# preiter93/ndrustfft

Hardware: AMD Instinct MI355X
Metric: GFFT-points/s, batched 1-D C2C FFT f64 along the contiguous axis (+ achieved HBM GB/s vs roofline) (higher is better)
Workload: dtype f64

## Files before the change

### include/ndfft_mi355x.h

```cpp
#ifndef NDFFT_MI355X_H
#define NDFFT_MI355X_H

#include <stddef.h>
#include <stdint.h>

#ifdef __cplusplus
extern "C" {
#endif

#define NDFFT_ABI_VERSION 1
#define NDFFT_ABI_MINOR 6

typedef enum {
    NDFFT_OK = 0,
    NDFFT_ERR_INVALID_ARG = 1,
    NDFFT_ERR_SIZE_MISMATCH = 2,
    NDFFT_ERR_SHAPE_MISMATCH = 3,
    NDFFT_ERR_AXIS = 4,
    NDFFT_ERR_UNSUPPORTED = 5,
    NDFFT_ERR_HIP = 6,
    NDFFT_ERR_NO_DEVICE = 7,
    NDFFT_ERR_ALLOC = 8
} ndfft_status;

typedef enum { NDFFT_F32 = 0, NDFFT_F64 = 1 } ndfft_dtype;

typedef enum {
    NDFFT_KIND_C2C = 0,
    NDFFT_KIND_R2C = 1,
    NDFFT_KIND_DCT = 2
} ndfft_kind;

typedef enum {
    NDFFT_OP_C2C_FWD = 0,
    NDFFT_OP_C2C_INV = 1,
    NDFFT_OP_R2C = 2,
    NDFFT_OP_C2R = 3,
    NDFFT_OP_DCT1 = 4,
    NDFFT_OP_DCT2 = 5,
    NDFFT_OP_DCT3 = 6,
    NDFFT_OP_DCT4 = 7
} ndfft_op;

typedef enum { NDFFT_NORM_NONE = 0, NDFFT_NORM_DEFAULT = 1, NDFFT_NORM_SCALE = 2 } ndfft_norm;
// ... 70 lines not shown
```

### include/ndfft_mi355x_ext.h

```cpp
#ifndef NDFFT_MI355X_EXT_H
#define NDFFT_MI355X_EXT_H

#include "ndfft_mi355x.h"

#ifdef __cplusplus
extern "C" {
#endif

int ndfft_exec_weighted_device(const ndfft_plan *plan, int op, const void *d_in, void *d_out, int ndim,
                               const int64_t *shape_in, const int64_t *stride_in,
                               const int64_t *shape_out, const int64_t *stride_out,
                               int axis, const void *d_weights, size_t n_weights, void *stream);

#define NDFFT_FILTER_NO_FUSE 1
int ndfft_exec_filter_device(const ndfft_plan *plan, const void *d_in, void *d_out, int ndim,
                             const int64_t *shape, const int64_t *stride_in, const int64_t *stride_out, int axis,
                             const void *d_weights, size_t n_weights, int norm, double scale, int flags, void *stream);

int ndfft_exec_dct_filter_device(const ndfft_plan *plan, const void *d_in, void *d_out, int ndim,
                                 const int64_t *shape, const int64_t *stride_in, const int64_t *stride_out, int axis,
                                 const void *d_weights, size_t n_weights, int norm, double scale, int flags, void *stream);

#ifdef __cplusplus
}
#endif
#endif
```

### ndrustfft_amd/_lib.py

```python
import ctypes
import os

_HERE = os.path.dirname(os.path.abspath(__file__))
LIB_PATH = os.environ.get("NDFFT_MI355X_LIB") or os.path.join(_HERE, "csrc", "libndfft_mi355x.so")

OK, ERR_INVALID_ARG, ERR_SIZE_MISMATCH, ERR_SHAPE_MISMATCH, ERR_AXIS, ERR_UNSUPPORTED, ERR_HIP, ERR_NO_DEVICE, ERR_ALLOC = range(9)
F32, F64 = 0, 1
KIND_C2C, KIND_R2C, KIND_DCT = 0, 1, 2
OP_C2C_FWD, OP_C2C_INV, OP_R2C, OP_C2R, OP_DCT1, OP_DCT2, OP_DCT3, OP_DCT4 = range(8)
NORM_NONE, NORM_DEFAULT, NORM_SCALE = 0, 1, 2
INPUT_AUTO, INPUT_CACHED, INPUT_COLD = 0, 1, 2

SYMBOLS = [
    "ndfft_abi_version", "ndfft_abi_minor", "ndfft_last_error", "ndfft_device_count", "ndfft_set_device",
    "ndfft_plan_create", "ndfft_plan_retain", "ndfft_plan_destroy", "ndfft_plan_n", "ndfft_plan_kind",
    "ndfft_plan_dtype", "ndfft_plan_lane_len_in", "ndfft_plan_lane_len_out",
    "ndfft_exec", "ndfft_exec_device", "ndfft_exec_sharded", "ndfft_exec_sharded_device", "ndfft_last_path", "ndfft_explain_plan",
    "ndfft_dev_alloc", "ndfft_dev_free", "ndfft_dev_upload", "ndfft_dev_download", "ndfft_dev_sync",
    "ndfft_release_workspace", "ndfft_host_alloc", "ndfft_host_free", "ndfft_set_input_hint", "ndfft_host_forget", "ndfft_host_reg_cache", "ndfft_last_input_policy",
    "ndfft_documented_switches", "ndfft_reload_switches", "ndfft_jit_prebuild",
]
EXT_SYMBOLS = ["ndfft_exec_weighted_device"]
FILTER_SYMBOLS = ["ndfft_exec_filter_device"]
FILTER_NO_FUSE = 1
DCT_FILTER_SYMBOLS = ["ndfft_exec_dct_filter_device"]


_loaded = []


class NdfftError(RuntimeError):
    def __init__(self, status, msg):
        super().__init__(msg)
        self.status = status


class Panic(NdfftError):
    """A condition on which the reference panics (size / axis / Zip mismatch); message text matches."""


class Library:
    def __init__(self, path=LIB_PATH):
        if not os.path.exists(path):
            raise ImportError(
                f"{path} not found: build it with `make -C ndrustfft_amd/csrc` (or __graft_entry__.build()). "
                "ndrustfft_amd has no CPU fallback.")
        self.path = path
        L = self.c = ctypes.CDLL(path)
        _loaded.append(self)
        vp, i32, sz, i64p, dbl = ctypes.c_void_p, ctypes.c_int, ctypes.c_size_t, ctypes.c_void_p, ctypes.c_double
        L.ndfft_abi_version.restype = i32
        L.ndfft_abi_minor.restype = i32
        L.ndfft_last_error.restype = ctypes.c_char_p
        L.ndfft_last_path.restype = ctypes.c_char_p
        L.ndfft_explain_plan.argtypes = [ctypes.c_int, ctypes.c_int, ctypes.c_size_t, ctypes.c_char_p, ctypes.c_size_t]
        L.ndfft_explain_plan.restype = ctypes.c_int
        L.ndfft_device_count.restype = i32
        L.ndfft_set_device.argtypes = [i32]
# ... 16 lines not shown
        L.ndfft_dev_upload.argtypes = [vp, vp, sz]
        L.ndfft_dev_download.argtypes = [vp, vp, sz]
        L.ndfft_dev_sync.argtypes = [vp]
        L.ndfft_release_workspace.argtypes = []; L.ndfft_release_workspace.restype = ctypes.c_int
        L.ndfft_host_alloc.argtypes = [ctypes.POINTER(vp), ctypes.c_size_t]; L.ndfft_host_alloc.restype = ctypes.c_int
        L.ndfft_host_free.argtypes = [vp]; L.ndfft_host_free.restype = ctypes.c_int
        L.ndfft_set_input_hint.argtypes = [i32]; L.ndfft_set_input_hint.restype = i32
        L.ndfft_host_forget.argtypes = [vp]; L.ndfft_host_forget.restype = i32
        L.ndfft_host_reg_cache.argtypes = [sz]; L.ndfft_host_reg_cache.restype = i32
        L.ndfft_last_input_policy.argtypes = []; L.ndfft_last_input_policy.restype = i32
        L.ndfft_documented_switches.argtypes = [ctypes.c_char_p, sz]; L.ndfft_documented_switches.restype = i32
        L.ndfft_reload_switches.argtypes = []; L.ndfft_reload_switches.restype = i32
        ip = ctypes.POINTER(ctypes.c_int)
        try:
            L.ndfft_jit_prebuild.argtypes = [ctypes.c_char_p, ctypes.c_char_p, i32, i32, ip, ip, ip]; L.ndfft_jit_prebuild.restype = i32
        except AttributeError:
            if not os.environ.get("NDFFT_MI355X_LIB"):
                raise
        try:
            L.ndfft_exec_weighted_device.argtypes = [vp, i32, vp, vp, i32, i64p, i64p, i64p, i64p, i32, vp, sz, vp]; L.ndfft_exec_weighted_device.restype = i32
        except AttributeError:
            if not os.environ.get("NDFFT_MI355X_LIB"):
                raise
        try:
            L.ndfft_exec_filter_device.argtypes = [vp, vp, vp, i32, i64p, i64p, i64p, i32, vp, sz, i32, dbl, i32, vp]; L.ndfft_exec_filter_device.restype = i32
        except AttributeError:
            if not os.environ.get("NDFFT_MI355X_LIB"):
                raise
        try:
            L.ndfft_exec_dct_filter_device.argtypes = [vp, vp, vp, i32, i64p, i64p, i64p, i32, vp, sz, i32, dbl, i32, vp]; L.ndfft_exec_dct_filter_device.restype = i32
        except AttributeError:
            if not os.environ.get("NDFFT_MI355X_LIB"):
                raise

    def check(self, status):
        if status == OK:
            return
        msg = self.c.ndfft_last_error().decode() or f"ndfft status {status}"
        if status in (ERR_SIZE_MISMATCH, ERR_SHAPE_MISMATCH, ERR_AXIS):
            raise Panic(status, msg)
        raise NdfftError(status, msg)

    def last_path(self):
        return self.c.ndfft_last_path().decode()

    def reload_switches(self):
        self.check(self.c.ndfft_reload_switches())

    def jit_prebuild(self, manifest, out_dir, first=0, stride=1):
        b, p, f = ctypes.c_int(0), ctypes.c_int(0), ctypes.c_int(0)
        self.check(self.c.ndfft_jit_prebuild(os.fsencode(manifest), os.fsencode(out_dir), first, stride, ctypes.byref(b), ctypes.byref(p), ctypes.byref(f)))
        return b.value, p.value, f.value

    def documented_switches(self):
        buf = ctypes.create_string_buffer(4096)
        self.c.ndfft_documented_switches(buf, len(buf))
        return buf.value.decode().split()

    def last_input_policy(self):
        return int(self.c.ndfft_last_input_policy())

    def explain_plan(self, kind, dtype, n):
        buf = ctypes.create_string_buffer(4096)
        need = self.c.ndfft_explain_plan(kind, dtype, n, buf, len(buf))
        if need < 0:
            raise NdfftError(-need, self.c.ndfft_last_error().decode())
        return buf.value.decode()


_default = None


def default():
    global _default
    if _default is None:
        _default = Library()
    return _default
```

### ndrustfft_amd/csrc/device_common.h

```cpp
#pragma once
#ifndef __HIPCC_RTC__
#include <hip/hip_runtime.h>
#include <stdint.h>
#else
typedef __hip_internal::int64_t int64_t;
typedef __hip_internal::int32_t int32_t;
typedef __hip_internal::uint32_t uint32_t;
typedef __hip_internal::uint64_t uint64_t;
#endif

namespace ndfft {

template <typename T> struct vec2;
typedef float ndfft_c32 __attribute__((ext_vector_type(2)));
template <> struct vec2<float> { using type = ndfft_c32; };
template <> struct vec2<double> { using type = double2; };
template <typename T> using cpx = typename vec2<T>::type;

template <typename T> __host__ __device__ inline cpx<T> mk(T a, T b) { cpx<T> r; r.x = a; r.y = b; return r; }
template <typename C> __host__ __device__ inline C cadd(C a, C b) { a.x += b.x; a.y += b.y; return a; }
template <typename C> __host__ __device__ inline C csub(C a, C b) { a.x -= b.x; a.y -= b.y; return a; }
template <typename C> __host__ __device__ inline C cmul(C a, C b) {
    C r; r.x = a.x * b.x - a.y * b.y; r.y = a.x * b.y + a.y * b.x; return r;
}
__host__ __device__ inline ndfft_c32 cadd(ndfft_c32 a, ndfft_c32 b) { return a + b; }
__host__ __device__ inline ndfft_c32 csub(ndfft_c32 a, ndfft_c32 b) { return a - b; }
__host__ __device__ inline ndfft_c32 cmul(ndfft_c32 a, ndfft_c32 b) { const ndfft_c32 bs = {-b.y, b.x}; return a.xx * b + a.yy * bs; }
template <typename C> __host__ __device__ inline C cconj(C a) { a.y = -a.y; return a; }
template <typename C> __host__ __device__ inline C cmul_mi(C a) { C r; r.x = a.y; r.y = -a.x; return r; }

enum GenOp : int {
    G_C2C_FWD = 0, G_C2C_INV,
    G_R2C_EVEN, G_R2C_ODD, G_C2R_EVEN, G_C2R_ODD,
    G_DCT1,
    G_DCT2_EVEN, G_DCT2_ODD, G_DCT3_EVEN, G_DCT3_ODD,
    G_DCT4_EVEN, G_DCT4_ODD
};

struct Pow2Args {
    const void *in; void *out;
    int64_t nlanes;
    int64_t pitch_in, pitch_out;
    int32_t inverse;
    double scale;
    const void *twp;
    const void *twlo = nullptr, *twhi = nullptr;
    int32_t logB = 0, f1 = 1;
    int32_t xcd_chunk = 0;
    int32_t stream_in = -1;
};

struct WaveArgs {
    const void *in; void *out;
    int64_t total;
    int32_t inverse;
    double scale;
    const void *tw;
    int32_t xcd_chunk;
};

struct TinyArgs {
    const void *in; void *out;
    int64_t nlanes;
    int64_t inner;
    int64_t outer_in, outer_out;
    int64_t lane_in, lane_out;
    int64_t elem_in, elem_out;
    int32_t inverse;
    double scale;
    const void *mat = nullptr;
};

struct RegRealArgs {
    TinyArgs t;
    const void *aux1, *aux2;
};

__device__ __forceinline__ unsigned xcd_block(unsigned b, unsigned nblk, int chunk) {
    if (chunk <= 0) return b;
    const unsigned grp = 8u * (unsigned)chunk;
    const unsigned g = b / grp;
    if ((g + 1) * grp > nblk) return b;
    const unsigned r = b - g * grp;
    return g * grp + (r & 7u) * (unsigned)chunk + (r >> 3);
}

}
```

### ndrustfft_amd/csrc/exec.hip

```cpp
#include <algorithm>
#include <atomic>
#include <mutex>
#include <cstdio>
#include <cstdlib>
#include <cstring>
#include <map>
#include <string>
#include <type_traits>

#include "exec_internal.h"
#include "pow2_real.h"
#include "../../include/ndfft_mi355x_ext.h"

namespace ndfft {

static int kind_of_op(int op) {
    if (op == NDFFT_OP_C2C_FWD || op == NDFFT_OP_C2C_INV) return NDFFT_KIND_C2C;
    if (op == NDFFT_OP_R2C || op == NDFFT_OP_C2R) return NDFFT_KIND_R2C;
    return NDFFT_KIND_DCT;
}

static int gen_op_of(int op, int n, int *slot) {
    *slot = CFG_MAIN;
    switch (op) {
// ... 155 lines not shown
    const size_t lds = generic_lds_bytes(lpb, pitch, csize, nbuf);
    int threads = 64; while (threads < lpb * fft_tpl && threads < maxthr) threads <<= 1;
    if (col) while (threads < 4 * lpb && threads < maxthr) threads <<= 1;
    if (inplace && threads < lpb * fft_tpl) return fail(NDFFT_ERR_INVALID_ARG, "internal: in-place thread map");
    fft_tpl = std::min(fft_tpl, threads);
    int io_tpl = 1; while (io_tpl < std::max(a.n_in, a.n_out) && io_tpl < threads) io_tpl <<= 1;
    a.fft_tpl_log = 0; while ((1 << a.fft_tpl_log) < fft_tpl) ++a.fft_tpl_log;
    a.io_tpl_log = 0; while ((1 << a.io_tpl_log) < io_tpl) ++a.io_tpl_log;
    set_last_path(col ? "generic_col" : (P.xs == 1 || P.xlen == 1) && (P.ys == 1 || P.ylen == 1) ? "generic_row" : "generic_strided");
    return launch_generic<T>(a, threads, lds, stream);
}

struct ThreadWs {
    std::map<int, DeviceWs> dev;
    void release_all() {
        if (dev.empty()) return;
        int cur = 0;
        if (hipGetDevice(&cur) != hipSuccess) { (void)hipGetLastError(); dev.clear(); return; }
        for (auto &kv : dev) { if (hipSetDevice(kv.first) == hipSuccess) { (void)hipDeviceSynchronize(); kv.second.release(); } }
        (void)hipSetDevice(cur);
        dev.clear();
    }
    ~ThreadWs() { release_all(); }
};
static thread_local ThreadWs g_tws;
int current_ws(DeviceWs **out) {
    int dev = 0;
    NDFFT_HIP(hipGetDevice(&dev));
    *out = &g_tws.dev[dev];
    return NDFFT_OK;
}
static thread_local int g_input_hint = NDFFT_INPUT_AUTO;
static thread_local int g_last_policy = -1;
void reset_last_policy() { g_last_policy = -1; }
static bool F_nt_ok(int F) { return F >= 64; }
static int row_load_policy(const void *in, size_t bytes, const void *out, size_t out_bytes);
int c2c_row_load_policy(const void *in, const void *out, size_t bytes) { return row_load_policy(in, bytes, out, bytes); }
static int row_load_policy(const void *in, size_t bytes, const void *out, size_t out_bytes) {
    const int force = sw().stream_loads;
    DeviceWs *ws;
    if (current_ws(&ws)) return -1;
    int pol = force >= 0 ? (force != 0) : g_input_hint == NDFFT_INPUT_CACHED ? 0 : g_input_hint == NDFFT_INPUT_COLD ? 1 : ws->mall.decide(in, bytes);
    const bool nt = pol >= 0 ? pol != 0 : stream_loads_for(bytes);
    g_last_policy = nt ? 1 : 0;
    ws->mall.note_read(in, bytes);
    ws->mall.note_write(out, out_bytes);
    return nt ? 1 : 0;
}
int get_scratch(int which, hipStream_t s, size_t bytes, void **out) {
    DeviceWs *ws;
    int rc = current_ws(&ws);
    if (rc) return rc;
    Scratch &sc = ws->scratch[which][s];
    if (bytes > sc.cap) {
        if (sc.p) { NDFFT_HIP(hipStreamSynchronize(s)); NDFFT_HIP(hipFree(sc.p)); sc.p = nullptr; sc.cap = 0; }
        NDFFT_HIP(hipMalloc(&sc.p, bytes));
        sc.cap = bytes;
    }
    *out = sc.p;
    return NDFFT_OK;
}

static int jit_rc(int rc) { return rc == NDFFT_ERR_UNSUPPORTED ? kDeclined : rc; }
static int took(int rc, const char *path) {
    if (rc != kDeclined) set_last_path(path);
    return rc;
}

static int transpose_batched(const void *in, void *out, int64_t batch, int64_t rows, int64_t cols, int64_t ld_in, int64_t ld_out,
                             int64_t bs_in, int64_t bs_out, int esz, hipStream_t s) {
    for (int64_t b0 = 0; b0 < batch; b0 += 32768) {
        const int64_t nb = std::min<int64_t>(32768, batch - b0);
        int rc = launch_transpose((const char *)in + b0 * bs_in * esz, (char *)out + b0 * bs_out * esz, nb, rows, cols, ld_in, ld_out,
                                  bs_in, bs_out, esz, s);
        if (rc) return rc;
    }
    return NDFFT_OK;
// ... 444 lines not shown
        return kDeclined;
    const FftConfig &c = k.plan->cfg[k.slot];
    const DevConfig &d = k.dt.cfg[k.slot];
    int f1, f2;
    if (c.big || !d.wave_tw || !regfft_factor(c.F, &f1, &f2) || !(k.L.dense || k.L.cols)) return kDeclined;
    RegRealArgs ra;
    ra.t = tiny_args(k, 0, d.wave_tw); ra.aux1 = d.aux1; ra.aux2 = d.aux2;
    return took(jit_rc(launch_jit_regreal(k.plan->dtype, k.gop, k.n, f1, f2, k.L.dense, ra, k.stream)), k.L.dense ? "regreal_row" : "regreal_col");
}

static int route_tinymat(const Call &k) {
    if (!(k.plan->kind != NDFFT_KIND_C2C && k.n >= 2 && k.n <= 16 && k.P.b.size() <= 2 && tiny_enabled())) return kDeclined;
    const bool r2c = k.plan->kind == NDFFT_KIND_R2C;
    const int q = r2c ? (k.P.op == NDFFT_OP_R2C ? 0 : 1) : k.P.op - NDFFT_OP_DCT1;
    const void *mat = k.dt.cfg[CFG_MAIN].tinymat[q];
    if (!mat) return kDeclined;
    set_last_path(k.L.dense ? "tinymat_row" : k.L.cols ? "tinymat_col" : "tinymat_strided");
    const TinyArgs a = tiny_args(k, 0, mat);
    const int shape = r2c ? q : 2;
    return k.f32() ? launch_tinymat_f32(k.n, shape, k.L.dense, a, k.stream) : launch_tinymat_f64(k.n, shape, k.L.dense, a, k.stream);
}

static Pow2Args c2c_row_args(const Call &k) {
    Pow2Args a;
    a.in = k.in; a.out = k.out; a.nlanes = k.P.nlanes; a.pitch_in = k.L.pitch_in; a.pitch_out = k.L.pitch_out;
    a.inverse = k.P.op == NDFFT_OP_C2C_INV; a.scale = k.P.scale; a.twp = k.dt.cfg[CFG_MAIN].twp;
    return a;
}

static bool pow2_rows_eligible(const Call &k) { return k.plan->kind == NDFFT_KIND_C2C && k.plan->cfg[CFG_MAIN].pow2 && k.L.rows; }
static int route_pow2_rows(const Call &k) {
    if (!pow2_rows_eligible(k)) return kDeclined;
    Pow2Args a = c2c_row_args(k);
    if (k.L.dense) a.stream_in = c2c_row_load_policy(k.in, k.out, (size_t)k.P.nlanes * k.plan->n * 2 * real_size(k.plan->dtype));
    set_last_path("pow2_reg");
    return launch_pow2(k.plan->dtype, k.n, a, k.stream);
}

static int route_jit_rows(const Call &k) {
    if (!(k.plan->kind == NDFFT_KIND_C2C && k.plan->cfg[CFG_MAIN].jit && k.L.rows && k.P.nlanes * (int64_t)k.n >= (1 << 17))) return kDeclined;
    const Pow2Args a = c2c_row_args(k);
    const size_t bytes_c = (size_t)k.P.nlanes * k.plan->n * 2 * real_size(k.plan->dtype);
    const int pol = k.L.dense ? c2c_row_load_policy(k.in, k.out, bytes_c) : -1;
    const int nt = (pol >= 0 ? pol != 0 : stream_loads_for(bytes_c)) ? 3 : 1;
    const int rc = took(jit_rc(launch_jit_c2c(k.plan->dtype, k.plan->cfg[CFG_MAIN].jitcfg, nt, a, k.stream)), "jit_reg");
    if (rc == kDeclined && sw().jit_verbose) fprintf(stderr, "ndfft: jit_reg declined n = %zu\n", k.plan->n);
    return rc;
}

struct Engine {
    bool use_jit, use_rader, use_blue, use_plain, col_alt;
    bool row, col;
};

template <typename T>
static int narrow_tiles(const Call &k) {
    const FftConfig &c = k.plan->cfg[k.slot];
    const DevConfig &d = k.dt.cfg[k.slot];
    RealArgs<T> a{};
    a.in = k.in; a.out = k.out; a.nlanes = k.P.nlanes;
    a.xcd_remap = 1;
    a.n = k.n; a.F = c.F; a.n_in = (int)k.P.xlen; a.n_out = (int)k.P.ylen; a.scale = (T)k.P.scale;
    a.inner = k.L.inner; a.outer_in = k.L.outer_in; a.outer_out = k.L.outer_out;
    a.elem_in = k.P.xs; a.elem_out = k.P.ys;
    a.aux1 = (const cpx<T> *)d.aux1; a.aux2 = (const cpx<T> *)d.aux2; a.twp = (const cpx<T> *)d.twp_narrow;
    const int rc = launch_pow2_real_narrow<T>(k.gop, a, k.stream);
    set_last_path("pow2_col_xcd");
// ... 137 lines not shown
int dispatch(const Problem &P, const void *d_in, void *d_out, hipStream_t stream) {
    const DevTables *dt;
    int rc = get_dev_tables(P.plan, &dt);
    if (rc) return rc;
    const Call k(P, d_in, d_out, stream, *dt);
    for (int (*route)(const Call &) : {route_wave, route_tiny, route_reg, route_regreal, route_tinymat, route_pow2_rows, route_jit_rows,
                                       route_real_engine, route_long, route_transposed, route_packed})
        if ((rc = route(k)) != kDeclined) return rc;
    return k.f32() ? dispatch_generic<float>(P, d_in, d_out, *dt, stream) : dispatch_generic<double>(P, d_in, d_out, *dt, stream);
}

}

using namespace ndfft;

extern "C" {

int ndfft_exec_device(const ndfft_plan *plan, int op, const void *d_in, void *d_out, int ndim,
                      const int64_t *shape_in, const int64_t *stride_in, const int64_t *shape_out,
                      const int64_t *stride_out, int axis, int norm, double scale, void *stream) {
    clear_err();
    reset_last_policy();
    Problem P;
    bool nothing;
    int rc = prepare(plan, op, ndim, shape_in, stride_in, shape_out, stride_out, axis, norm, scale, P, nothing);
    if (rc || nothing) return rc;
    if (!d_in || !d_out) return fail(NDFFT_ERR_INVALID_ARG, "null array pointer");
    const size_t r = real_size(plan->dtype);
    return dispatch_peeled(P, (const char *)d_in, (char *)d_out, op_in_cplx(op) ? 2 * r : r, op_out_cplx(op) ? 2 * r : r,
                           (hipStream_t)stream);
}

int ndfft_last_input_policy(void) { return g_last_policy; }

int ndfft_set_input_hint(int hint) {
    clear_err();
    if (hint < NDFFT_INPUT_AUTO || hint > NDFFT_INPUT_COLD) return fail(NDFFT_ERR_INVALID_ARG, "bad input hint");
    g_input_hint = hint;
    return NDFFT_OK;
}

int ndfft_release_workspace(void) {
    clear_err();
    g_tws.release_all();
    shard_release_all();
    return NDFFT_OK;
}

}

#ifndef NDFFT_HOST_UNIT
#include "host.hip"
#endif
#ifndef NDFFT_COMPOSE_UNIT
#include "compose.hip"
#endif
```

### ndrustfft_amd/csrc/exec_internal.h

```cpp
#pragma once
#include "engine.h"

namespace ndfft {

struct BatchDim { int64_t shape, sin, sout; };

struct Problem {
    const ndfft_plan *plan;
    int op;
    int64_t xlen, ylen;
    int64_t xs, ys;
    std::vector<BatchDim> b;
    int64_t nlanes;
    double scale;
    int keep_out = 0;
    int stream_in = 0;
    int no_xcd_map = 0;
    int makhoul_out = 0;
};

inline size_t real_size(int dtype) { return dtype == NDFFT_F32 ? 4 : 8; }
inline bool op_in_cplx(int op) { return op == NDFFT_OP_C2C_FWD || op == NDFFT_OP_C2C_INV || op == NDFFT_OP_C2R; }
inline bool op_out_cplx(int op) { return op == NDFFT_OP_C2C_FWD || op == NDFFT_OP_C2C_INV || op == NDFFT_OP_R2C; }

int prepare(const ndfft_plan *plan, int op, int ndim, const int64_t *shape_in, const int64_t *stride_in, const int64_t *shape_out,
            const int64_t *stride_out, int axis, int norm, double scale, Problem &P, bool &nothing);
int dispatch_peeled(Problem &P, const char *d_in, char *d_out, size_t ein, size_t eout, hipStream_t stream);

int dispatch(const Problem &P, const void *d_in, void *d_out, hipStream_t stream);
int prefixed(const char *prefix, int rc);
int get_scratch(int which, hipStream_t s, size_t bytes, void **out);
int c2c_row_load_policy(const void *in, const void *out, size_t bytes);
void reset_last_policy();

struct Layout {
    bool rows;
    bool dense;
    bool cols;
    int64_t pitch_in, pitch_out;
    int64_t inner;
    int64_t lane_in, lane_out;
    int64_t outer_in, outer_out;
    explicit Layout(const Problem &P) {
        const size_t nb = P.b.size();
        rows = P.xs == 1 && P.ys == 1 && nb <= 1;
        pitch_in = nb ? P.b[0].sin : P.xlen; pitch_out = nb ? P.b[0].sout : P.ylen;
        dense = rows && pitch_in == P.xlen && pitch_out == P.ylen;
        cols = nb && P.b.back().sin == 1 && P.b.back().sout == 1;
        inner = nb ? P.b.back().shape : 1;
        lane_in = nb ? P.b.back().sin : 0; lane_out = nb ? P.b.back().sout : 0;
        outer_in = nb == 2 ? P.b[0].sin : 0; outer_out = nb == 2 ? P.b[0].sout : 0;
    }
};

constexpr int kDeclined = -1;

struct Scratch { void *p = nullptr; size_t cap = 0; };
struct Staging {
    void *p = nullptr; size_t cap = 0;
    int reserve(size_t bytes) {
        if (bytes <= cap) return NDFFT_OK;
        if (p) (void)hipFree(p);
        p = nullptr; cap = 0;
        NDFFT_HIP(hipMalloc(&p, bytes));
        cap = bytes;
// ... 2 lines not shown
    void release() { if (p) (void)hipFree(p); p = nullptr; cap = 0; }
};
struct PinnedBuf {
    void *p = nullptr; size_t cap = 0;
    int reserve(size_t bytes) {
        if (bytes <= cap) return NDFFT_OK;
        if (p) (void)hipHostFree(p);
        p = nullptr; cap = 0;
        NDFFT_HIP(hipHostMalloc(&p, bytes, hipHostMallocDefault));
        cap = bytes;
        return NDFFT_OK;
    }
    void release() { if (p) (void)hipHostFree(p); p = nullptr; cap = 0; }
};
struct Pipe {
    hipStream_t h2d = nullptr, cmp = nullptr, d2h = nullptr;
    std::vector<hipEvent_t> up, done, down;
    bool ok = false;
    void sync_all() { if (ok) { (void)hipStreamSynchronize(h2d); (void)hipStreamSynchronize(cmp); (void)hipStreamSynchronize(d2h); } }
    void release() {
        if (!ok) return;
        sync_all();
        for (auto *v : {&up, &done, &down}) { for (hipEvent_t e : *v) (void)hipEventDestroy(e); v->clear(); }
        (void)hipStreamDestroy(h2d); (void)hipStreamDestroy(cmp); (void)hipStreamDestroy(d2h);
        h2d = cmp = d2h = nullptr; ok = false;
    }
};
struct MallModel {
    enum State { READ = 0, OUT_SMALL = 1, OUT_COLD = 2 };
    struct Entry { uintptr_t lo, hi; uint64_t stamp; int state; };
    std::vector<Entry> e;
    uint64_t clock = 0;
    static constexpr uint64_t kCap = (uint64_t)256 << 20, kSmallOut = (uint64_t)64 << 20;
    Entry *find(const void *p, size_t bytes) {
        const uintptr_t lo = (uintptr_t)p, hi = lo + bytes;
        for (auto &x : e) if (lo < x.hi && x.lo < hi) return &x;
        return nullptr;
    }
    int decide(const void *in, size_t bytes) {
        const Entry *x = find(in, bytes);
        if (!x) return -1;
        if (x->state == OUT_COLD) return 1;
        if (bytes > kCap) return clock == x->stamp ? -1 : 1;
        return clock - x->stamp + bytes <= kCap ? 0 : 1;
    }
    void put(const void *p, size_t bytes, int state, bool through_cache) {
        const uintptr_t lo = (uintptr_t)p, hi = lo + bytes;
        for (size_t i = 0; i < e.size();) { if (lo < e[i].hi && e[i].lo < hi) e.erase(e.begin() + i); else ++i; }
        if (through_cache) clock += bytes;
        if (e.size() >= 32) e.erase(e.begin());
        e.push_back({lo, hi, clock, state});
    }
    void note_read(const void *p, size_t bytes) { put(p, bytes, READ, true); }
    void note_write(const void *p, size_t bytes) { if (bytes <= kSmallOut) put(p, bytes, OUT_SMALL, true); else put(p, bytes, OUT_COLD, false); }
};
struct DeviceWs {
    MallModel mall;
    std::map<hipStream_t, Scratch> scratch[9];
    Staging stage_in, stage_out;
    PinnedBuf bounce_in[3], bounce_out[3];
    Pipe pipe;
    void release() {
        pipe.release();
        for (auto &m : scratch) { for (auto &kv : m) if (kv.second.p) (void)hipFree(kv.second.p); m.clear(); }
        stage_in.release(); stage_out.release();
        for (auto &b : bounce_in) b.release();
// ... 7 lines not shown
```

### ndrustfft_amd/csrc/kernels_pow2.hip

```cpp
#include <algorithm>
#include <cstdlib>

#include "pow2_config.h"

namespace ndfft {

bool pow2_supported(int dtype, int n) {
    (void)dtype;
    switch (n) {
#define NDFFT_CASE(N_, TPL_, ...) case N_: return true;
        NDFFT_POW2_CONFIGS_F64(NDFFT_CASE)
#undef NDFFT_CASE
        default: return false;
    }
}

void pow2_build_twiddles(int dtype, int n, HostTable &out) {
    switch (n) {
#define NDFFT_CASE(N_, TPL_, ...) \
    case N_: if (dtype == NDFFT_F32) build_tw<Pow2Cfg<float, N_>::RL>(out); else build_tw<Pow2Cfg<double, N_>::RL>(out); break;
        NDFFT_POW2_CONFIGS_F64(NDFFT_CASE)
#undef NDFFT_CASE
        default: break;
    }
}

int xcd_chunk_for(size_t block_bytes, int64_t nblk) {
    const long kb = NDFFT_DEV_INT("NDFFT_XCD_CHUNK_KB", 512);
    if (kb <= 0 || block_bytes == 0) return 0;
    if (block_bytes >= ((size_t)256 << 10)) return 0;
    int64_t c = (int64_t)((size_t)kb * 1024 / block_bytes);
    if (c < 1) c = 1;
    if (nblk < 16 * c) return 0;
    return (int)std::min<int64_t>(c, 1 << 20);
}
bool stream_loads_for(size_t in_bytes) {
    const int force = sw().stream_loads;
    if (force >= 0) return force != 0;
    return in_bytes > ((size_t)384 << 20);
}

static int psplit_override() { return (int)NDFFT_DEV_INT("NDFFT_PSPLIT", 0); }

template <typename T, int N, int NT, int VEC, int FL, int PS> static int launch_inst_ps(const Pow2Args &a0, hipStream_t s) {
    constexpr int TPL = Pow2Cfg<T, N>::TPL, LPB = lpb_for(TPL);
    static_assert((FL & ~8) == 0, "callers choose the fused four-step form only; every other flag is pow2_config.h's choice");
    using K = Pow2RowKernel<T, N, NT, VEC, (FL & 8) != 0, PS>;
    NDFFT_ENSURE_LDS_ATTR((k_pow2<K>));
    const int64_t nblk = (a0.nlanes + LPB - 1) / LPB;
    if (nblk <= 0) return NDFFT_OK;
    if (nblk > 0x7fffffffLL) return fail(NDFFT_ERR_UNSUPPORTED, "too many lanes for one launch");
    Pow2Args a = a0;
    a.xcd_chunk = xcd_chunk_for((size_t)LPB * N * sizeof(cpx<T>), nblk);
    const size_t pad = (size_t)NDFFT_DEV_INT("NDFFT_POW2_LDS_PAD_KB", 0) << 10;
    hipLaunchKernelGGL(k_pow2<K>, dim3((unsigned)nblk), dim3(K::THREADS), std::min(K::LDS_BYTES + pad, (size_t)160 * 1024), s, a);
    NDFFT_HIP(hipGetLastError());
    return NDFFT_OK;
}
template <typename T, int N, int NT, int VEC, int FL = 0> static int launch_inst(const Pow2Args &a, hipStream_t s) {
    if constexpr (N >= 8192) {
        const int ov = psplit_override();
        const int ps = ov == 1 || ov == 2 ? ov : Pow2PSplit<T, N>::value;
        return ps == 2 ? launch_inst_ps<T, N, NT, VEC, FL, 2>(a, s) : launch_inst_ps<T, N, NT, VEC, FL, 1>(a, s);
    } else {
        return launch_inst_ps<T, N, NT, VEC, FL, 1>(a, s);
    }
}
template <typename T, int N, int NT, int VEC, int FL = 0> static int launch_one(const Pow2Args &a, hipStream_t s) {
    static_assert(NT == 1, "callers name the store policy; the load policy is chosen here");
    const bool nt_in = a.stream_in >= 0 ? a.stream_in != 0 : stream_loads_for((size_t)a.nlanes * N * sizeof(cpx<T>));
    if (nt_in) return launch_inst<T, N, 3, VEC, FL>(a, s);
    return launch_inst<T, N, 1, VEC, FL>(a, s);
}

template <int N> static int launch_f32(bool vec_ok, bool fused, const Pow2Args &a, hipStream_t s) {
    if constexpr (f32_can_vec2<N>()) {
        if (vec_ok) return fused ? launch_one<float, N, 1, 2, 8>(a, s) : launch_one<float, N, 1, 2>(a, s);
    }
    return fused ? launch_one<float, N, 1, 1, 8>(a, s) : launch_one<float, N, 1, 1>(a, s);
}

int launch_pow2(int dtype, int n, const Pow2Args &a, hipStream_t s) {
    const bool vec_ok = a.pitch_in % 2 == 0 && a.pitch_out % 2 == 0 && ((uintptr_t)a.in % 16) == 0 && ((uintptr_t)a.out % 16) == 0;
    const bool fused = a.twlo != nullptr;
    switch (n) {
#define NDFFT_CASE(N_, TPL_, ...)                                                               \
    case N_:                                                                                    \
        if (dtype == NDFFT_F64) return fused ? launch_one<double, N_, 1, 1, 8>(a, s) : launch_one<double, N_, 1, 1>(a, s); \
        return launch_f32<N_>(vec_ok, fused, a, s);
        NDFFT_POW2_CONFIGS_F64(NDFFT_CASE)
#undef NDFFT_CASE
        default: return fail(NDFFT_ERR_UNSUPPORTED, "pow2 kernel: unsupported n");
    }
}

}

#ifndef NDFFT_FILTER_UNIT
#include "kernels_filter.hip"
#endif
```

### ndrustfft_amd/csrc/plan.hip

```cpp
#include <algorithm>
#include <cmath>
#include <cstdlib>
#include <cstring>
#include <tuple>

#include "engine.h"

namespace ndfft {

static thread_local std::string g_err;
static thread_local const char *g_path = "";

int fail(int code, const std::string &msg) { g_err = msg; return code; }
void set_last_path(const char *p) { g_path = p; }
const char *last_path() { return g_path; }
const std::string &last_err() { return g_err; }
void clear_err() { g_err.clear(); }

static const long double kPiL = 3.14159265358979323846264338327950288L;

static void unit(HostTable &t, unsigned long long num, unsigned long long den) {
    num %= den;
    long double ang = 2.0L * kPiL * (long double)num / (long double)den;
    t.re.push_back(cosl(ang));
// ... 537 lines not shown

namespace ndfft {
namespace {
std::atomic<const Switches *> g_sw{nullptr};
std::mutex g_sw_mu;
const Switches *parse_switches() {
    Switches *S = new Switches();
    auto str = [](const char *name, bool &set, std::string &v) { const char *e = getenv(name); set = e != nullptr; v = e ? e : ""; };
    auto on = [](const char *name, bool def) { const char *e = getenv(name); return e ? e[0] != '0' : def; };
    auto one = [](const char *name) { const char *e = getenv(name); return e && e[0] == '1'; };
    auto num = [](const char *name, long def, long lo, long hi) {
        const char *e = getenv(name);
        if (!e) return def;
        char *end = nullptr;
        const long v = strtol(e, &end, 10);
        if (end == e) return def;
        return std::min(hi, std::max(lo, v));
    };
    if (const char *e = getenv("NDFFT_JIT")) S->jit = e[0] == '0' ? 0 : !strcmp(e, "cached") ? 2 : 1;
    str("NDFFT_JIT_CACHE", S->jit_cache_set, S->jit_cache);
    str("NDFFT_JIT_PREBUILT", S->jit_prebuilt_set, S->jit_prebuilt);
    S->jit_verbose = getenv("NDFFT_JIT_VERBOSE") != nullptr;
    if (const char *e = getenv("NDFFT_JIT_DUMP_SRC")) S->jit_dump_src = e;
    if (const char *e = getenv("XDG_CACHE_HOME")) S->xdg_cache_home = e;
    if (const char *e = getenv("HOME")) S->home = e;
    S->wave = on("NDFFT_WAVE", true); S->tiny = on("NDFFT_TINY", true); S->plain = on("NDFFT_PLAIN", true); S->blue = on("NDFFT_BLUE", true);
    S->rader = on("NDFFT_RADER", true); S->colsplit = on("NDFFT_COLSPLIT", true); S->fourstep2 = on("NDFFT_FOURSTEP2", true);
    S->real_fourstep = (int)num("NDFFT_REAL_FOURSTEP", 1, 0, 2);
    if (const char *e = getenv("NDFFT_FS_DIRECT")) S->fs_direct = e[0] == '1' ? 1 : 0;
    S->narrow_dct = one("NDFFT_NARROW_DCT");
    S->rfs_c2r_tile = on("NDFFT_RFS_C2R_TILE", true);
    S->rfs_logn1 = (int)num("NDFFT_RFS_LOGN1", 0, 0, 11);
    S->cs_chunk_mb = (int)num("NDFFT_CS_CHUNK_MB", 144, 0, 1 << 20);
    S->stream_loads = (int)num("NDFFT_STREAM_LOADS", -1, -1, 1);
    if (const char *e = getenv("NDFFT_HOST_PIPE")) S->host_pipe = e[0] == '1' ? 1 : e[0] == '0' ? 0 : -1;
    S->host_reg_cache_mb = num("NDFFT_HOST_REG_CACHE_MB", 0, 0, 1L << 22);
    S->copy_threads = (int)num("NDFFT_COPY_THREADS", 0, 0, 64);
    S->shard_chunk_kb = num("NDFFT_SHARD_CHUNK_KB", 0, 1, 1L << 24);
    S->shard_force_remote = one("NDFFT_SHARD_FORCE_REMOTE");
    return S;
}
}
const Switches &sw() {
    const Switches *p = g_sw.load(std::memory_order_acquire);
    if (__builtin_expect(p != nullptr, 1)) return *p;
    std::lock_guard<std::mutex> g(g_sw_mu);
    p = g_sw.load(std::memory_order_relaxed);
    if (!p) { p = parse_switches(); g_sw.store(p, std::memory_order_release); }
    return *p;
}
void reload_switches() {
    std::lock_guard<std::mutex> g(g_sw_mu);
    g_sw.store(parse_switches(), std::memory_order_release);
}
}

extern "C" {

int ndfft_abi_version(void) { return NDFFT_ABI_VERSION; }
int ndfft_abi_minor(void) { return NDFFT_ABI_MINOR; }
int ndfft_reload_switches(void) { ndfft::reload_switches(); return NDFFT_OK; }
int ndfft_documented_switches(char *buf, size_t cap) {
    static const char *const names[] = {NDFFT_DOCUMENTED_SWITCHES};
    std::string s;
    for (const char *n : names) { s += n; s += '\n'; }
    if (buf && cap) { const size_t k = std::min(cap - 1, s.size()); memcpy(buf, s.data(), k); buf[k] = 0; }
    return (int)s.size();
}
// ... 144 lines not shown
```

### ndrustfft_amd/csrc/pow2_kernel.h

```cpp
#pragma once
#include "butterflies.h"
#ifndef __HIPCC_RTC__
#include "engine.h"
#include <cmath>
#endif

namespace ndfft {

template <int... Rs> struct RadixList {
    static constexpr int NP = sizeof...(Rs);
    static constexpr int at(int i) { constexpr int r[NP] = {Rs...}; return r[i]; }
    static constexpr int ns(int i) { int s = 1; for (int p = 0; p < i; ++p) s *= at(p); return s; }
    static constexpr int twoff(int i) { int o = 0; for (int p = 1; p < i; ++p) o += (at(p) - 1) * ns(p); return o; }
};

#ifndef NDFFT_PHI_SHIFT
#define NDFFT_PHI_SHIFT 4
#endif
__device__ __forceinline__ int phi(int p) { return p + (p >> NDFFT_PHI_SHIFT); }
template <int STRIDE> __device__ __forceinline__ int phi_at(int base, int pbase, int r) {
    if constexpr (STRIDE % (1 << NDFFT_PHI_SHIFT) == 0) return pbase + r * (STRIDE + (STRIDE >> NDFFT_PHI_SHIFT));
    else return phi(base + r * STRIDE);
}
template <int Ns> __device__ __forceinline__ int kmod(int j) {
// ... 200 lines not shown
                        const int j = jof<P>(t, q), k = kmod<Ns>(j), o = (j - k) * R + k - ps * (N / 2), po = phi(o);
                        if ((FULL || j < NB) && (PSPLIT == 1 || (j < NB / 2) == (ps == 0))) {
#pragma unroll
                            for (int r = 0; r < R; ++r) s[phi_at<Ns>(o, po, r)] = v[q * R + r];
                        }
                    }
                    xbar<PREF>();
#pragma unroll
                    for (int q = 0; q < NBF2; ++q) {
                        const int j = jof<P + 1>(t, q), pj = phi(j);
                        if (FULL2 || j < NB2) {
#pragma unroll
                            for (int r = 0; r < R2 / PSPLIT; ++r) {
                                const cpx<T> x = s[phi_at<NB2>(j, pj, r)];
                                if constexpr (PSPLIT == 2) {
                                    if (ps == 0) { keep[q * (R2 / 2) + r] = x; continue; }
                                }
                                v[q * R2 + r + ps * (R2 / 2)] = x;
                            }
                        }
                    }
                }
                if constexpr (PSPLIT == 2) {
#pragma unroll
                    for (int q = 0; q < NBF2; ++q)
#pragma unroll
                        for (int r = 0; r < R2 / 2; ++r) v[q * R2 + r] = keep[q * (R2 / 2) + r];
                }
            }
            passes_w<P + 1>(v, twp, lds, t, wpre);
        }
    }

    static __device__ __forceinline__ void run(const Pow2Args &a) {
        extern __shared__ __attribute__((aligned(16))) char smem[];
        const int t = threadIdx.x % TPL, ll = threadIdx.x / TPL;
        const int64_t lane = (int64_t)xcd_block(blockIdx.x, gridDim.x, a.xcd_chunk) * LPB + ll;
        const bool live = lane < a.nlanes;
        const cpx<T> *in = (const cpx<T> *)a.in + (live ? lane : 0) * a.pitch_in;
        cpx<T> *out = (cpx<T> *)a.out + (live ? lane : 0) * a.pitch_out;
        char *lds = smem + (size_t)ll * LANE_LDS * (HALF ? sizeof(T) : 2 * sizeof(T));
        cpx<T> v[E];
        {
            constexpr int R0 = RL::at(0), NB0 = N / R0, NBF0 = slots(0);
            if constexpr (VEC == 2) {
                static_assert(NBF0 % 2 == 0 && full(0) && full(RL::NP - 1), "VEC=2 needs an even number of whole butterfly rounds in the first and last pass");
#pragma unroll
                for (int q = 0; q < NBF0; q += 2)
#pragma unroll
                    for (int r = 0; r < R0; ++r) {
                        const vec4f w = gload4<(NT & 2) != 0>((const float *)(in + jof<0>(t, q) + r * NB0));
                        v[q * R0 + r] = mk<T>(w.x, w.y); v[(q + 1) * R0 + r] = mk<T>(w.z, w.w);
                    }
            } else {
#pragma unroll
                for (int q = 0; q < NBF0; ++q)
                    if (full(0) || t + q * TPL < NB0) {
#pragma unroll
                        for (int r = 0; r < R0; ++r) v[q * R0 + r] = gload<T, (NT & 2) != 0>(in + t + q * TPL + r * NB0);
                    }
            }
        }
        cpx<T> w[DERIVE ? E : 1];
        if constexpr (DERIVE && RL::NP > 1 && !(FLAGS & 1)) load_tw<1>(w, (const cpx<T> *)a.twp, t);
        if (a.inverse) {
#pragma unroll
            for (int i = 0; i < E; ++i) v[i].y = -v[i].y;
        }
        if constexpr ((FLAGS & 8) != 0) {
            constexpr int R0 = RL::at(0), NB0 = N / R0, NBF0 = slots(0);
            const int k1 = (int)(lane % a.f1), mask = (1 << a.logB) - 1;
            const cpx<T> *lo = (const cpx<T> *)a.twlo, *hi = (const cpx<T> *)a.twhi;
#pragma unroll
            for (int q = 0; q < NBF0; ++q)
                if (full(0) || jof<0>(t, q) < NB0) {
#pragma unroll
                    for (int r = 0; r < R0; ++r) {
                        const int m = (jof<0>(t, q) + r * NB0) * k1;
                        v[q * R0 + r] = cmul(v[q * R0 + r], cmul(hi[m >> a.logB], lo[m & mask]));
                    }
                }
        }
        if constexpr (DERIVE) passes_w<0>(v, (const cpx<T> *)a.twp, lds, t, w);
        else passes<0>(v, (const cpx<T> *)a.twp, lds, t);
        if (!live) return;
        constexpr int RL_ = RL::at(RL::NP - 1), NBL = N / RL_, NBFL = slots(RL::NP - 1);
        if (a.inverse) {
            const T sc = (T)a.scale;
#pragma unroll
            for (int i = 0; i < E; ++i) { v[i].x *= sc; v[i].y *= -sc; }
        }
        if constexpr (VEC == 2) {
            static_assert(NBFL % 2 == 0, "VEC=2 needs an even number of butterflies per thread in the last pass");
#pragma unroll
// ... 38 lines not shown
```

Before: 185.3.

## Keep a budgeted share of streamed input lanes cached in MALL

When the MALL model decides the input should be streamed with non-temporal loads, it now estimates from reuse distance and a budget what fraction (out of 64) of input blocks could stay resident in the last-level cache. A new kernel instance picks per lane-block whether to use cached or non-temporal loads through a hashed block selector. The aim is to recover cache hits on repeated inputs that exceed the cache without polluting it entirely. It adds a kernel instantiation and per-lane branching, and relies on a heuristic reuse model that may misjudge residency.

```diff
diff --git a/include/ndfft_mi355x.h b/include/ndfft_mi355x.h
--- a/include/ndfft_mi355x.h
+++ b/include/ndfft_mi355x.h
@@ -9,7 +9,7 @@
 #endif
 
 #define NDFFT_ABI_VERSION 1
-#define NDFFT_ABI_MINOR 6
+#define NDFFT_ABI_MINOR 7
 
 typedef enum {
     NDFFT_OK = 0,
diff --git a/include/ndfft_mi355x_ext.h b/include/ndfft_mi355x_ext.h
--- a/include/ndfft_mi355x_ext.h
+++ b/include/ndfft_mi355x_ext.h
@@ -24,4 +24,7 @@
 #ifdef __cplusplus
 }
 #endif
+
+#include "ndfft_mi355x_keep.h"
+
 #endif
diff --git a/include/ndfft_mi355x_keep.h b/include/ndfft_mi355x_keep.h
--- /dev/null
+++ b/include/ndfft_mi355x_keep.h
@@ -0,0 +1,17 @@
+#ifndef NDFFT_MI355X_KEEP_H
+#define NDFFT_MI355X_KEEP_H
+
+#include "ndfft_mi355x.h"
+
+#ifdef __cplusplus
+extern "C" {
+#endif
+
+int ndfft_last_input_keep(void);
+int ndfft_set_keep_budget(int mib);
+int ndfft_force_input_keep(int keep64);
+
+#ifdef __cplusplus
+}
+#endif
+#endif
diff --git a/ndrustfft_amd/_lib.py b/ndrustfft_amd/_lib.py
--- a/ndrustfft_amd/_lib.py
+++ b/ndrustfft_amd/_lib.py
@@ -24,6 +24,7 @@
 FILTER_SYMBOLS = ["ndfft_exec_filter_device"]
 FILTER_NO_FUSE = 1
 DCT_FILTER_SYMBOLS = ["ndfft_exec_dct_filter_device"]
+KEEP_SYMBOLS = ["ndfft_last_input_keep", "ndfft_set_keep_budget", "ndfft_force_input_keep"]
 
 
 _loaded = []
@@ -106,6 +107,13 @@
         except AttributeError:
             if not os.environ.get("NDFFT_MI355X_LIB"):
                 raise
+        try:
+            L.ndfft_last_input_keep.argtypes = []; L.ndfft_last_input_keep.restype = i32
+            L.ndfft_set_keep_budget.argtypes = [i32]; L.ndfft_set_keep_budget.restype = i32
+            L.ndfft_force_input_keep.argtypes = [i32]; L.ndfft_force_input_keep.restype = i32
+        except AttributeError:
+            if not os.environ.get("NDFFT_MI355X_LIB"):
+                raise
 
     def check(self, status):
         if status == OK:
@@ -134,6 +142,15 @@
     def last_input_policy(self):
         return int(self.c.ndfft_last_input_policy())
 
+    def last_input_keep(self):
+        return int(self.c.ndfft_last_input_keep()) if hasattr(self.c, "ndfft_last_input_keep") else 0
+
+    def set_keep_budget(self, mib):
+        self.check(self.c.ndfft_set_keep_budget(mib))
+
+    def force_input_keep(self, keep64):
+        self.check(self.c.ndfft_force_input_keep(keep64))
+
     def explain_plan(self, kind, dtype, n):
         buf = ctypes.create_string_buffer(4096)
         need = self.c.ndfft_explain_plan(kind, dtype, n, buf, len(buf))
diff --git a/ndrustfft_amd/csrc/device_common.h b/ndrustfft_amd/csrc/device_common.h
--- a/ndrustfft_amd/csrc/device_common.h
+++ b/ndrustfft_amd/csrc/device_common.h
@@ -48,6 +48,7 @@
     int32_t logB = 0, f1 = 1;
     int32_t xcd_chunk = 0;
     int32_t stream_in = -1;
+    int32_t keep64 = 0, keep_shift = 0;
 };
 
 struct WaveArgs {
@@ -85,4 +86,10 @@
     return g * grp + (r & 7u) * (unsigned)chunk + (r >> 3);
 }
 
+__host__ __device__ __forceinline__ bool keep_block(int64_t lane, int keep64, int shift) {
+    const int64_t blk = lane >> shift;
+    const unsigned b = (unsigned)(blk + (blk >> 6)) & 63u;
+    return (int)(((b & 7u) << 3) | (b >> 3)) < keep64;
 }
+
+}
diff --git a/ndrustfft_amd/csrc/exec.hip b/ndrustfft_amd/csrc/exec.hip
--- a/ndrustfft_amd/csrc/exec.hip
+++ b/ndrustfft_amd/csrc/exec.hip
@@ -211,17 +211,29 @@
 }
 static thread_local int g_input_hint = NDFFT_INPUT_AUTO;
 static thread_local int g_last_policy = -1;
-void reset_last_policy() { g_last_policy = -1; }
+static thread_local int g_last_keep = 0;
+static thread_local int g_keep_budget_mb = -1;
+static thread_local int g_keep_force = -1;
+void reset_last_policy() { g_last_policy = -1; g_last_keep = 0; }
 static bool F_nt_ok(int F) { return F >= 64; }
-static int row_load_policy(const void *in, size_t bytes, const void *out, size_t out_bytes);
-int c2c_row_load_policy(const void *in, const void *out, size_t bytes) { return row_load_policy(in, bytes, out, bytes); }
-static int row_load_policy(const void *in, size_t bytes, const void *out, size_t out_bytes) {
+static int row_load_policy(const void *in, size_t bytes, const void *out, size_t out_bytes, int *keep64 = nullptr, bool grant = true);
+int c2c_row_load_policy(const void *in, const void *out, size_t bytes, int *keep64, bool grant) { return row_load_policy(in, bytes, out, bytes, keep64, grant); }
+static int row_load_policy(const void *in, size_t bytes, const void *out, size_t out_bytes, int *keep64, bool grant) {
     const int force = sw().stream_loads;
     DeviceWs *ws;
     if (current_ws(&ws)) return -1;
+    const bool model = force < 0 && g_input_hint == NDFFT_INPUT_AUTO;
     int pol = force >= 0 ? (force != 0) : g_input_hint == NDFFT_INPUT_CACHED ? 0 : g_input_hint == NDFFT_INPUT_COLD ? 1 : ws->mall.decide(in, bytes);
     const bool nt = pol >= 0 ? pol != 0 : stream_loads_for(bytes);
     g_last_policy = nt ? 1 : 0;
+    if (keep64) {
+        const int kb = g_keep_budget_mb >= 0 ? g_keep_budget_mb : (int)NDFFT_DEV_INT("NDFFT_KEEP_BUDGET_MB", -1);
+        const int kf = g_keep_force >= 0 ? g_keep_force : (int)std::min<long>(64, NDFFT_DEV_INT("NDFFT_KEEP64", -1));
+        const uint64_t budget = kb >= 0 ? (uint64_t)kb << 20 : MallModel::kKeepBudget;
+        int k = grant && model && pol != 0 && budget ? ws->mall.share(in, bytes, budget) : 0;
+        if (kf >= 0 && nt) k = kf;
+        *keep64 = g_last_keep = k;
+    }
     ws->mall.note_read(in, bytes);
     ws->mall.note_write(out, out_bytes);
     return nt ? 1 : 0;
@@ -732,7 +744,7 @@
 static int route_pow2_rows(const Call &k) {
     if (!pow2_rows_eligible(k)) return kDeclined;
     Pow2Args a = c2c_row_args(k);
-    if (k.L.dense) a.stream_in = c2c_row_load_policy(k.in, k.out, (size_t)k.P.nlanes * k.plan->n * 2 * real_size(k.plan->dtype));
+    if (k.L.dense) a.stream_in = c2c_row_load_policy(k.in, k.out, (size_t)k.P.nlanes * k.plan->n * 2 * real_size(k.plan->dtype), &a.keep64, k.plan->dtype == NDFFT_F64);
     set_last_path("pow2_reg");
     return launch_pow2(k.plan->dtype, k.n, a, k.stream);
 }
@@ -936,6 +948,19 @@
 }
 
 int ndfft_last_input_policy(void) { return g_last_policy; }
+int ndfft_last_input_keep(void) { return g_last_keep; }
+int ndfft_set_keep_budget(int mib) {
+    clear_err();
+    if (mib > (1 << 20)) return fail(NDFFT_ERR_INVALID_ARG, "keep budget beyond 2^20 MiB");
+    g_keep_budget_mb = mib < 0 ? -1 : mib;
+    return NDFFT_OK;
+}
+int ndfft_force_input_keep(int keep64) {
+    clear_err();
+    if (keep64 > 64) return fail(NDFFT_ERR_INVALID_ARG, "kept share beyond 64");
+    g_keep_force = keep64 < 0 ? -1 : keep64;
+    return NDFFT_OK;
+}
 
 int ndfft_set_input_hint(int hint) {
     clear_err();
diff --git a/ndrustfft_amd/csrc/exec_internal.h b/ndrustfft_amd/csrc/exec_internal.h
--- a/ndrustfft_amd/csrc/exec_internal.h
+++ b/ndrustfft_amd/csrc/exec_internal.h
@@ -30,7 +30,7 @@
 int dispatch(const Problem &P, const void *d_in, void *d_out, hipStream_t stream);
 int prefixed(const char *prefix, int rc);
 int get_scratch(int which, hipStream_t s, size_t bytes, void **out);
-int c2c_row_load_policy(const void *in, const void *out, size_t bytes);
+int c2c_row_load_policy(const void *in, const void *out, size_t bytes, int *keep64 = nullptr, bool grant = true);
 void reset_last_policy();
 
 struct Layout {
@@ -99,6 +99,13 @@
     std::vector<Entry> e;
     uint64_t clock = 0;
     static constexpr uint64_t kCap = (uint64_t)256 << 20, kSmallOut = (uint64_t)64 << 20;
+    static constexpr uint64_t kKeepBudget = (uint64_t)192 << 20;
+    int share(const void *in, size_t bytes, uint64_t budget) {
+        const Entry *x = find(in, bytes);
+        if (!x || x->state != READ || bytes == 0) return 0;
+        const uint64_t d = clock - x->stamp + bytes;
+        return (int)std::min<uint64_t>(63, 64 * budget / d);
+    }
     Entry *find(const void *p, size_t bytes) {
         const uintptr_t lo = (uintptr_t)p, hi = lo + bytes;
         for (auto &x : e) if (lo < x.hi && x.lo < hi) return &x;
diff --git a/ndrustfft_amd/csrc/kernels_pow2.hip b/ndrustfft_amd/csrc/kernels_pow2.hip
--- a/ndrustfft_amd/csrc/kernels_pow2.hip
+++ b/ndrustfft_amd/csrc/kernels_pow2.hip
@@ -52,6 +52,10 @@
     if (nblk > 0x7fffffffLL) return fail(NDFFT_ERR_UNSUPPORTED, "too many lanes for one launch");
     Pow2Args a = a0;
     a.xcd_chunk = xcd_chunk_for((size_t)LPB * N * sizeof(cpx<T>), nblk);
+    constexpr size_t lane_bytes = (size_t)N * sizeof(cpx<T>);
+    a.keep_shift = 0;
+    for (size_t b = lane_bytes; b < ((size_t)64 << 10); b <<= 1) ++a.keep_shift;
+    if ((NT & 4) == 0) a.keep64 = 0;
     const size_t pad = (size_t)NDFFT_DEV_INT("NDFFT_POW2_LDS_PAD_KB", 0) << 10;
     hipLaunchKernelGGL(k_pow2<K>, dim3((unsigned)nblk), dim3(K::THREADS), std::min(K::LDS_BYTES + pad, (size_t)160 * 1024), s, a);
     NDFFT_HIP(hipGetLastError());
@@ -69,6 +73,9 @@
 template <typename T, int N, int NT, int VEC, int FL = 0> static int launch_one(const Pow2Args &a, hipStream_t s) {
     static_assert(NT == 1, "callers name the store policy; the load policy is chosen here");
     const bool nt_in = a.stream_in >= 0 ? a.stream_in != 0 : stream_loads_for((size_t)a.nlanes * N * sizeof(cpx<T>));
+    if constexpr (FL == 0) {
+        if (nt_in && a.keep64 > 0 && a.pitch_in == N) return launch_inst<T, N, 7, VEC, FL>(a, s);
+    }
     if (nt_in) return launch_inst<T, N, 3, VEC, FL>(a, s);
     return launch_inst<T, N, 1, VEC, FL>(a, s);
 }
diff --git a/ndrustfft_amd/csrc/plan.hip b/ndrustfft_amd/csrc/plan.hip
--- a/ndrustfft_amd/csrc/plan.hip
+++ b/ndrustfft_amd/csrc/plan.hip
@@ -593,8 +593,7 @@
     S->rfs_c2r_tile = on("NDFFT_RFS_C2R_TILE", true);
     S->rfs_logn1 = (int)num("NDFFT_RFS_LOGN1", 0, 0, 11);
     S->cs_chunk_mb = (int)num("NDFFT_CS_CHUNK_MB", 144, 0, 1 << 20);
-    S->stream_loads = (int)num("NDFFT_STREAM_LOADS", -1, -1, 1);
-    if (const char *e = getenv("NDFFT_HOST_PIPE")) S->host_pipe = e[0] == '1' ? 1 : e[0] == '0' ? 0 : -1;
+    S->stream_loads = (int)num("NDFFT_STREAM_LOADS", -1, -1, 1);    if (const char *e = getenv("NDFFT_HOST_PIPE")) S->host_pipe = e[0] == '1' ? 1 : e[0] == '0' ? 0 : -1;
     S->host_reg_cache_mb = num("NDFFT_HOST_REG_CACHE_MB", 0, 0, 1L << 22);
     S->copy_threads = (int)num("NDFFT_COPY_THREADS", 0, 0, 64);
     S->shard_chunk_kb = num("NDFFT_SHARD_CHUNK_KB", 0, 1, 1L << 24);
diff --git a/ndrustfft_amd/csrc/pow2_kernel.h b/ndrustfft_amd/csrc/pow2_kernel.h
--- a/ndrustfft_amd/csrc/pow2_kernel.h
+++ b/ndrustfft_amd/csrc/pow2_kernel.h
@@ -256,6 +256,27 @@
         }
     }
 
+    template <bool NTL> static __device__ __forceinline__ void load_lane(cpx<T> (&v)[E], const cpx<T> *in, int t) {
+        constexpr int R0 = RL::at(0), NB0 = N / R0, NBF0 = slots(0);
+        if constexpr (VEC == 2) {
+            static_assert(NBF0 % 2 == 0 && full(0) && full(RL::NP - 1), "VEC=2 needs an even number of whole butterfly rounds in the first and last pass");
+#pragma unroll
+            for (int q = 0; q < NBF0; q += 2)
+#pragma unroll
+                for (int r = 0; r < R0; ++r) {
+                    const vec4f w = gload4<NTL>((const float *)(in + jof<0>(t, q) + r * NB0));
+                    v[q * R0 + r] = mk<T>(w.x, w.y); v[(q + 1) * R0 + r] = mk<T>(w.z, w.w);
+                }
+        } else {
+#pragma unroll
+            for (int q = 0; q < NBF0; ++q)
+                if (full(0) || t + q * TPL < NB0) {
+#pragma unroll
+                    for (int r = 0; r < R0; ++r) v[q * R0 + r] = gload<T, NTL>(in + t + q * TPL + r * NB0);
+                }
+        }
+    }
+
     static __device__ __forceinline__ void run(const Pow2Args &a) {
         extern __shared__ __attribute__((aligned(16))) char smem[];
         const int t = threadIdx.x % TPL, ll = threadIdx.x / TPL;
@@ -265,25 +286,12 @@
         cpx<T> *out = (cpx<T> *)a.out + (live ? lane : 0) * a.pitch_out;
         char *lds = smem + (size_t)ll * LANE_LDS * (HALF ? sizeof(T) : 2 * sizeof(T));
         cpx<T> v[E];
-        {
-            constexpr int R0 = RL::at(0), NB0 = N / R0, NBF0 = slots(0);
-            if constexpr (VEC == 2) {
-                static_assert(NBF0 % 2 == 0 && full(0) && full(RL::NP - 1), "VEC=2 needs an even number of whole butterfly rounds in the first and last pass");
-#pragma unroll
-                for (int q = 0; q < NBF0; q += 2)
-#pragma unroll
-                    for (int r = 0; r < R0; ++r) {
-                        const vec4f w = gload4<(NT & 2) != 0>((const float *)(in + jof<0>(t, q) + r * NB0));
-                        v[q * R0 + r] = mk<T>(w.x, w.y); v[(q + 1) * R0 + r] = mk<T>(w.z, w.w);
-                    }
-            } else {
-#pragma unroll
-                for (int q = 0; q < NBF0; ++q)
-                    if (full(0) || t + q * TPL < NB0) {
-#pragma unroll
-                        for (int r = 0; r < R0; ++r) v[q * R0 + r] = gload<T, (NT & 2) != 0>(in + t + q * TPL + r * NB0);
-                    }
-            }
+        if constexpr ((NT & 4) != 0) {
+            static_assert((NT & 2) != 0, "a kept share is a form of the streaming-load instances");
+            if (keep_block(lane, a.keep64, a.keep_shift)) load_lane<false>(v, in, t);
+            else load_lane<true>(v, in, t);
+        } else {
+            load_lane<(NT & 2) != 0>(v, in, t);
         }
         cpx<T> w[DERIVE ? E : 1];
         if constexpr (DERIVE && RL::NP > 1 && !(FLAGS & 1)) load_tw<1>(w, (const cpx<T> *)a.twp, t);
```

Measured after the change: 192.7, median of 6. 4.0% higher.
